# mKaloer/TFServingCache

Measured on AMD Instinct MI355X. Metric: predict req/sec (whole node), higher is better.
Workload: dtype bf16; 1 GPU; model=resnet50_v1.5, global_batch=8, seq_len=224, parallelism=ring-sharded serving x1, mode=headline (lru), full=False, batch_per_request=8, threads=10, n_models=1000, model_repo=hardlinked copies of one SavedModel per family (content-dedup applies), provider=disk, pool_size=10, n_cold_loads=872, transport=real gRPC (native nghttp2 front-end) over TCP loopback, client_channels=1, hipgraph=True

## Files before the change

### tfservingcache_amd/engine/csrc/executor.cpp

```cpp
#include <torch/extension.h>

#include <hip/hip_runtime.h>

#include <c10/hip/HIPStream.h>

#include <cstdint>
#include <stdexcept>
#include <vector>

#include "kernels.h"

namespace tfsc {

enum CallKind : int {
  K_ELT_UNARY = 0,
  K_ELT_BINARY,
  K_BN_ACT,
  K_SOFTMAX,
  K_LAYERNORM,
  K_MEAN_LAST,
  K_MEAN_MID,
  K_POOL,
  K_TRANSPOSE,
  K_GATHER,
  K_PAD_NHWC,
  K_GEMM,
  K_BGEMM,
  K_IM2COL,
  K_CONV,
  K_PAD_LAST,
  K_ATTENTION,
  K_DEPTHWISE,
  K_GEMM_FP8,
  K_QUANT_FP8,
  K_CAST,
  K_ARGMAX_LAST,
  K_SCATTER,
  K_RESIZE,
  K_ZERO_INSERT,
};
// ... 237 lines not shown
}

struct PtrDesc {
  uint8_t tag;
  int32_t reg = 0;
  int64_t off = 0;
};

class CallTemplate {
 public:
  std::vector<Call> calls;
  std::vector<std::vector<PtrDesc>> descs;

  ExecPlan* instantiate(uintptr_t ws,
                        const std::vector<uintptr_t>& bases) const {
    std::vector<Call> out = calls;
    for (size_t i = 0; i < out.size(); ++i) {
      auto& ds = descs[i];
      auto& ptrs = out[i].ptrs;
      ptrs.resize(ds.size());
      for (size_t j = 0; j < ds.size(); ++j) {
        const PtrDesc& d = ds[j];
        if (d.tag == 0)
          ptrs[j] = intptr_t(ws) + d.off;
        else if (d.tag == 1)
          ptrs[j] = intptr_t(bases.at(size_t(d.reg))) + d.off;
        else
          ptrs[j] = 0;
      }
    }
    return new ExecPlan(out);
  }
};

}

namespace py = pybind11;

void register_fastpath(py::module_& mod);
void register_frontend(py::module_& mod);
void register_rest_frontend(py::module_& mod);

PYBIND11_MODULE(TORCH_EXTENSION_NAME, mod) {
  using tfsc::Call;
  using tfsc::ExecPlan;

  py::class_<ExecPlan>(mod, "ExecPlan")
      .def(py::init([](py::list calls) {
        std::vector<Call> cs;
        cs.reserve(calls.size());
        for (auto item : calls) {
          py::tuple t = item.cast<py::tuple>();
          Call c;
          c.kind = t[0].cast<int>();
          c.ptrs = t[1].cast<std::vector<intptr_t>>();
          c.ints = t[2].cast<std::vector<int64_t>>();
          c.floats = t[3].cast<std::vector<float>>();
          cs.push_back(std::move(c));
        }
        return new ExecPlan(cs);
      }))
      .def("run", &ExecPlan::run, py::call_guard<py::gil_scoped_release>())
      .def("capture", &ExecPlan::capture,
           py::call_guard<py::gil_scoped_release>())
      .def("run_graph", &ExecPlan::run_graph,
           py::call_guard<py::gil_scoped_release>())
// ... 35 lines not shown
        t->calls.reserve(calls.size());
        t->descs.reserve(calls.size());
        for (auto item : calls) {
          py::tuple tu = item.cast<py::tuple>();
          Call c;
          c.kind = tu[0].cast<int>();
          std::vector<tfsc::PtrDesc> ds;
          for (auto dd : tu[1].cast<py::list>()) {
            py::tuple dt = dd.cast<py::tuple>();
            tfsc::PtrDesc d;
            d.tag = uint8_t(dt[0].cast<int>());
            if (d.tag == 0) {
              d.off = dt[1].cast<int64_t>();
            } else if (d.tag == 1) {
              d.reg = dt[1].cast<int32_t>();
              d.off = dt[2].cast<int64_t>();
            }
            ds.push_back(d);
          }
          c.ints = tu[2].cast<std::vector<int64_t>>();
          c.floats = tu[3].cast<std::vector<float>>();
          t->calls.push_back(std::move(c));
          t->descs.push_back(std::move(ds));
        }
        return t;
      }));

  mod.def("instantiate_plan",
          [](const tfsc::CallTemplate& t, uintptr_t ws,
             const std::vector<uintptr_t>& bases) {
            return std::unique_ptr<ExecPlan>(t.instantiate(ws, bases));
          });

  register_fastpath(mod);
  register_frontend(mod);
  register_rest_frontend(mod);

  mod.attr("ELT_ADD") = int(tfsc::ELT_ADD);
  mod.attr("ELT_SUB") = int(tfsc::ELT_SUB);
  mod.attr("ELT_MUL") = int(tfsc::ELT_MUL);
  mod.attr("ELT_DIV") = int(tfsc::ELT_DIV);
  mod.attr("ELT_MAX") = int(tfsc::ELT_MAX);
  mod.attr("ELT_MIN") = int(tfsc::ELT_MIN);
  mod.attr("ELT_SQDIFF") = int(tfsc::ELT_SQDIFF);
  mod.attr("ELT_RELU") = int(tfsc::ELT_RELU);
  mod.attr("ELT_TANH") = int(tfsc::ELT_TANH);
  mod.attr("ELT_SIGMOID") = int(tfsc::ELT_SIGMOID);
  mod.attr("ELT_ERF") = int(tfsc::ELT_ERF);
  mod.attr("ELT_SQRT") = int(tfsc::ELT_SQRT);
  mod.attr("ELT_RSQRT") = int(tfsc::ELT_RSQRT);
  mod.attr("ELT_EXP") = int(tfsc::ELT_EXP);
  mod.attr("ELT_NEG") = int(tfsc::ELT_NEG);
  mod.attr("ELT_SQUARE") = int(tfsc::ELT_SQUARE);
  mod.attr("ELT_GELU") = int(tfsc::ELT_GELU);
  mod.attr("ELT_RELU6") = int(tfsc::ELT_RELU6);

  mod.attr("ACT_NONE") = int(tfsc::ACT_NONE);
  mod.attr("ACT_RELU") = int(tfsc::ACT_RELU);
  mod.attr("ACT_TANH") = int(tfsc::ACT_TANH);
  mod.attr("ACT_SIGMOID") = int(tfsc::ACT_SIGMOID);
  mod.attr("ACT_GELU") = int(tfsc::ACT_GELU);
  mod.attr("ACT_RELU6") = int(tfsc::ACT_RELU6);
}
```

### tfservingcache_amd/engine/csrc/kernels.h

```cpp
#pragma once

#include <hip/hip_runtime.h>
#include <cstdint>

namespace tfsc {

enum EltFn : int {
  ELT_ADD = 0, ELT_SUB, ELT_MUL, ELT_DIV, ELT_MAX, ELT_MIN, ELT_SQDIFF,
  ELT_RELU, ELT_TANH, ELT_SIGMOID, ELT_ERF, ELT_SQRT, ELT_RSQRT, ELT_EXP,
  ELT_NEG, ELT_SQUARE, ELT_GELU, ELT_RELU6,
};

enum Act : int { ACT_NONE = 0, ACT_RELU, ACT_TANH, ACT_SIGMOID, ACT_GELU,
                 ACT_RELU6 };

constexpr int MAX_DIMS = 6;

struct BcastArgs {
  int ndim;
  int64_t dims[MAX_DIMS];
  int64_t sa[MAX_DIMS];
  int64_t sb[MAX_DIMS];
};

// ... 43 lines not shown
                 const ushort* bias, const ushort* residual, ushort* C,
                 int64_t M, int64_t N, int64_t K, int act, float alpha);

void launch_batched_gemm(hipStream_t s, const ushort* A, const ushort* B,
                         ushort* C, int64_t bat, int64_t M, int64_t N,
                         int64_t K, int64_t strideA, int64_t strideB,
                         int64_t strideC, bool trans_b, float alpha);

void launch_conv_igemm(hipStream_t s, const ushort* x, const ushort* w,
                       const ushort* bias, const ushort* residual,
                       const ushort* zeros, ushort* y,
                       int N, int H, int W, int C, int Kc, int R, int S,
                       int sh, int sw, int pt, int pl, int Ho, int Wo,
                       int k_pad, int act);

void launch_im2col(hipStream_t s, const ushort* x, ushort* y,
                   int N, int H, int W, int C, int R, int S,
                   int sh, int sw, int pt, int pl, int Ho, int Wo,
                   int k_pad);

void launch_depthwise_conv(hipStream_t s, const ushort* x, const ushort* w,
                           const ushort* bias, ushort* y,
                           int N, int H, int W, int C, int R, int S,
                           int sh, int sw, int pt, int pl, int Ho, int Wo,
                           int act);

void launch_resize_nhwc(hipStream_t s, const ushort* x, ushort* y, int N,
                        int H, int W, int C, int Ho, int Wo, int mode,
                        bool align_corners, bool half_pixel_centers);

void launch_zero_insert_nhwc(hipStream_t s, const ushort* x, ushort* y,
                             int N, int h, int w, int C, int sh, int sw);

void launch_gemm_fp8(hipStream_t s, const uint8_t* A, const float* sa,
                     const uint8_t* B, const float* sb,
                     const ushort* bias, const ushort* residual,
                     ushort* C, int64_t M, int64_t N, int64_t K,
                     int act);

void launch_quant_rowwise(hipStream_t s, const ushort* x, uint8_t* q,
                          float* scales, int64_t M, int64_t K,
                          int64_t Kp);

void launch_attention(hipStream_t s, const ushort* Q, const ushort* K,
                      const ushort* V, ushort* O, int B, int S, int H,
                      int D_, float scale, const ushort* bias = nullptr,
                      int64_t bias_sb = 0, int64_t bias_sh = 0,
                      int64_t bias_sq = 0);

}
```

### tfservingcache_amd/engine/csrc/ops/ops_memory.hip

```cpp
#include "../common.h"
#include "../kernels.h"

#include <stdexcept>
#include <string>

namespace tfsc {

constexpr int TPB = 256;
constexpr int MAX_BLOCKS = 2048;

static inline int grid_for(int64_t n, int per_thread = 1) {
  int64_t blocks = ceil_div(n, int64_t(TPB) * per_thread);
  return int(blocks < MAX_BLOCKS ? (blocks > 0 ? blocks : 1) : MAX_BLOCKS);
}

TFSC_DEV float apply_unary(float v, int fn) {
  switch (fn) {
    case ELT_RELU: return v > 0.f ? v : 0.f;
    case ELT_TANH: return tanhf(v);
    case ELT_SIGMOID: return 1.f / (1.f + __expf(-v));
    case ELT_ERF: return erff(v);
    case ELT_SQRT: return sqrtf(v);
    case ELT_RSQRT: return rsqrtf(v);
    case ELT_EXP: return __expf(v);
// ... 969 lines not shown
  int64_t stride = (int64_t)gridDim.x * TPB;
  for (int64_t i = i0; i < n_out; i += stride) {
    int c = int(i % C);
    int64_t t = i / C;
    int wo = int(t % Wo); t /= Wo;
    int ho = int(t % Ho); int n = int(t / Ho);
    ushort v = 0;
    if (ho % sh == 0 && wo % sw == 0)
      v = x[(((int64_t)n * h + ho / sh) * w + wo / sw) * C + c];
    y[i] = v;
  }
}

void launch_zero_insert_nhwc(hipStream_t s, const ushort* x, ushort* y,
                             int N, int h, int w, int C, int sh, int sw) {
  if (N <= 0 || h <= 0 || w <= 0 || C <= 0 || sh <= 0 || sw <= 0)
    throw std::runtime_error(
        "zero_insert: every dimension and stride must be positive");
  int64_t Ho64 = (int64_t)(h - 1) * sh + 1, Wo64 = (int64_t)(w - 1) * sw + 1;
  if (Ho64 > INT32_MAX || Wo64 > INT32_MAX)
    throw std::runtime_error("zero_insert: output image too large");
  int Ho = int(Ho64), Wo = int(Wo64);
  if (C % 8 == 0 && aligned16(x, y)) {
    int64_t n_grp = (int64_t)N * Ho * Wo * (C / 8);
    hipLaunchKernelGGL(k_zero_insert_v8, dim3(grid_for(n_grp)), dim3(TPB),
                       0, s, x, y, N, h, w, C, sh, sw, Ho, Wo);
    return;
  }
  int64_t n_out = (int64_t)N * Ho * Wo * C;
  hipLaunchKernelGGL(k_zero_insert, dim3(grid_for(n_out)), dim3(TPB), 0, s,
                     x, y, N, h, w, C, sh, sw, Ho, Wo);
}

}
```

### tfservingcache_amd/engine/emit.py

```python
from __future__ import annotations

from dataclasses import dataclass
from typing import Dict, List, Optional, Tuple

import numpy as np

from .planner import Plan, PlanOp

ALIGN = 256

WS = ("ws",)

KINDS = frozenset({
    "ELT_UNARY", "ELT_BINARY", "BN_ACT", "SOFTMAX", "LAYERNORM",
    "MEAN_LAST", "MEAN_MID", "POOL", "TRANSPOSE", "GATHER", "PAD_NHWC",
    "GEMM", "BGEMM", "CONV", "PAD_LAST", "ATTENTION", "DEPTHWISE",
    "GEMM_FP8", "QUANT_FP8", "CAST", "ARGMAX_LAST", "SCATTER", "RESIZE",
    "ZERO_INSERT",
})

_ROWWISE = {"softmax": "SOFTMAX", "reduce_mean_last": "MEAN_LAST",
            "argmax_last": "ARGMAX_LAST"}

_ACT_CODE = {"none": 0, "relu": 1, "tanh": 2, "sigmoid": 3, "gelu": 4,
             "relu6": 5}

_ELT_CODE = {
    "add": 0, "sub": 1, "mul": 2, "div": 3, "max": 4, "min": 5,
    "sqdiff": 6, "relu": 7, "tanh": 8, "sigmoid": 9, "erf": 10,
    "sqrt": 11, "rsqrt": 12, "exp": 13, "neg": 14, "square": 15,
    "gelu": 16, "relu6": 17,
}


# ... 53 lines not shown
def blob_layout(plan: Plan) -> BlobLayout:
    slots: Dict[int, Tuple[int, int]] = {}
    int_idx: List[int] = []
    total = 0
    for t in plan.tensors:
        if t.kind != "weight" or t.weight is None:
            continue
        if t.weight.dtype in _INT_DTYPES:
            int_idx.append(t.idx)
        else:
            n = int(t.weight.size)
            slots[t.idx] = (total, n)
            total += _pad128(n)
    return BlobLayout(slots, total, int_idx)


@dataclass
class Template:
    shapes: List[Tuple[int, ...]]
    root: List[int]
    bufs: Dict[int, _BufInfo]
    total_bytes: int
    scratch_off: Dict[int, int]
    region_keys: List[tuple]
    calls: List[tuple]


def build_template(plan: Plan, batch: int, dtype: str) -> Template:
    e = _Emitter(plan, batch, dtype)
    e.plan_buffers()
    e.emit_calls()
    return Template(e.shapes, e.root, e.bufs, e.total_bytes,
                    e.scratch_off, e.region_keys, e.calls)


class _Emitter:
    def __init__(self, plan: Plan, batch: int, dtype: str):
        self.plan = plan
        self.batch = batch
        self.dtype = dtype
        self.layout = blob_layout(plan)
        self.shapes: List[Tuple[int, ...]] = [
            plan.resolve_shape(t.shape, batch) for t in plan.tensors]
        self.root = [t.alias_of if t.alias_of is not None else t.idx
                     for t in plan.tensors]
        for i, r in enumerate(self.root):
            seen = 0
            while plan.tensors[r].alias_of is not None and seen < 16:
                r = plan.tensors[r].alias_of
                seen += 1
            self.root[i] = r
        self.region_keys: List[tuple] = []
        self._seen = set()
        self.calls: List[tuple] = []

    def _buf_bytes(self, idx: int) -> int:
        esize = 4 if self.plan.tensors[idx].dtype == "i32" else 2
        return max(_numel(self.shapes[idx]) * esize, esize)

    def plan_buffers(self) -> None:
        plan = self.plan
        root = self.root
        live_end: Dict[int, int] = {}
        scratch_sizes: Dict[int, int] = {}

        n_ops = len(plan.ops)
# ... 387 lines not shown
```

### tfservingcache_amd/engine/gpu.py

```python
from __future__ import annotations

import contextlib
import logging
import threading
from typing import Dict, List, Optional, Tuple

import warnings

import numpy as np

from .emit import (WS, _pad64, _pad128, _pad256b, blob_layout,
                   build_template)
from .planner import Plan, is_sym, resolve_dim

warnings.filterwarnings(
    "ignore", message="The given NumPy array is not writable")

log = logging.getLogger("tfsc.gpu")

_torch = None
_ext = None
_import_lock = threading.Lock()


class GpuUnavailable(RuntimeError):
    pass


class ModelReleasedError(RuntimeError):
    """Raised when a request races a pool eviction; callers re-fetch."""


def _load_backend():
    global _torch, _ext
    with _import_lock:
        if _ext is not None:
            return _torch, _ext
        import torch
        if not torch.cuda.is_available():
            raise GpuUnavailable("no ROCm GPU visible")
        try:
            from . import _tfsc_engine as ext
        except ImportError as e:
            raise GpuUnavailable(
                "GPU present but the tfsc HIP engine extension is not "
                "built — run `PYTORCH_ROCM_ARCH=gfx950 python setup.py "
                f"build_ext --inplace` ({e})") from e
        _torch, _ext = torch, ext
        return torch, ext


# ... 184 lines not shown
_arena_order: List[tuple] = []


def _get_ctx_template(plan, bucket: int, dtype: str):
    with _tmpl_lock:
        key = (id(plan), bucket, dtype)
        ent = _ctx_templates.get(key)
        if ent is None or ent[0] is not plan:
            return None
        _tmpl_order.remove(key)
        _tmpl_order.append(key)
        return ent[1]


def _put_ctx_template(plan, bucket: int, dtype: str, tmpl) -> None:
    with _tmpl_lock:
        key = (id(plan), bucket, dtype)
        if key not in _ctx_templates:
            _tmpl_order.append(key)
        _ctx_templates[key] = (plan, tmpl)
        while len(_tmpl_order) > _TMPL_CAP:
            old = _tmpl_order.pop(0)
            _ctx_templates.pop(old, None)


def _get_transform_arena(plan, dtype: str):
    with _tmpl_lock:
        key = (id(plan), dtype)
        ent = _transform_arenas.get(key)
        if ent is None or ent[0] is not plan:
            return None
        _arena_order.remove(key)
        _arena_order.append(key)
        return ent[1], ent[2]


def _put_transform_arena(plan, dtype: str, entries, pinned) -> None:
    with _tmpl_lock:
        key = (id(plan), dtype)
        if key in _transform_arenas:
            return
        _arena_order.append(key)
        _transform_arenas[key] = (plan, entries, pinned)
        while len(_arena_order) > _ARENA_CAP:
            old = _arena_order.pop(0)
            _transform_arenas.pop(old, None)


def _call_template(ext, tmpl):
    index = {k: i for i, k in enumerate(tmpl.region_keys)}
    return ext.CallTemplate([
        (getattr(ext, "K_" + kind),
         [(2,) if d is None else (0, d[1]) if d[0] == WS
          else (1, index[d[0]], d[1]) for d in descs],
         ints, floats)
        for kind, descs, ints, floats in tmpl.calls])


class ExecContext:

    def __init__(self, gm: "GpuModel", batch: int):
        self.gm = gm
        self.batch = batch
        torch, ext = _load_backend()
        plan = gm.plan
        dev = gm.device

        cached = _get_ctx_template(plan, batch, gm.dtype)
        if cached is None:
            tmpl = build_template(plan, batch, gm.dtype)
            ctmpl = _call_template(ext, tmpl)
        else:
            tmpl, ctmpl = cached
        self.shapes = tmpl.shapes
        self.root = tmpl.root
        self.bufs = tmpl.bufs
        self.total_bytes = tmpl.total_bytes
        self.scratch_off = tmpl.scratch_off
        self.workspace = torch.empty(self.total_bytes,
                                     dtype=torch.uint8, device=dev)
        n_before = gm.n_transforms()
        bases = gm.region_bases(tmpl.region_keys)
        self.exec_plan = ext.instantiate_plan(
            ctmpl, self.workspace.data_ptr(), bases)
        self._from_template = cached is not None and \
            gm.n_transforms() == n_before
        if cached is None:
            _put_ctx_template(plan, batch, gm.dtype, (tmpl, ctmpl))
            gm.publish_transform_arena()
        self.captured = False
        self._views: Dict[int, object] = {}
        self.lock = threading.Lock()
        self.fast_id: Optional[int] = None
        self.stream = torch.cuda.Stream(device=dev)
        self._pinned_in: Dict[int, object] = {}
        self._pinned_out: Dict[int, object] = {}
        self._pin_raws: List[object] = []

    def capture_only(self):
        torch, _ = _load_backend()
        with torch.cuda.device(self.gm.device), \
                torch.cuda.stream(self.stream):
            try:
                with capture_guard.capture():
                    self.exec_plan.capture()
            except Exception:
                log.exception("hipGraph capture failed; staying eager")
            self.captured = True

    def view(self, idx: int):
        torch, _ = _load_backend()
        r = self.root[idx]
        v = self._views.get(idx)
        if v is not None:
            return v
        info = self.bufs[r]
        t = self.gm.plan.tensors[r]
        base = self.workspace[info.offset:info.offset + info.nbytes]
        if t.dtype == "i32":
            v = base.view(torch.int32)[:int(np.prod(self.shapes[idx]))]
        else:
            v = base.view(torch.bfloat16)[:int(np.prod(self.shapes[idx]))]
        v = v.view(self.shapes[idx])
        self._views[idx] = v
        return v

    def run(self, feeds: Dict[int, np.ndarray],
            fetch: List[int]) -> Dict[int, np.ndarray]:
        if self.fast_id is not None and self.fast_id >= 0:
            self.gm._fast.lock_ctx(self.fast_id)
            try:
                return self._run_inner(feeds, fetch)
            finally:
                self.gm._fast.unlock_ctx(self.fast_id)
        return self._run_inner(feeds, fetch)

    def _run_inner(self, feeds: Dict[int, np.ndarray],
                   fetch: List[int]) -> Dict[int, np.ndarray]:
        torch, _ = _load_backend()
        with torch.cuda.device(self.gm.device), \
# ... 57 lines not shown

class GpuModel:

    BUCKETS = (1, 2, 4, 8, 16, 32, 64)

    def __init__(self, plan: Plan, device: str = "cuda:0",
                 max_batch: int = 64, use_graphs: bool = True,
                 n_streams: int = 6, model_name: str = "",
                 model_version: int = 0, dtype: str = "bf16"):
        torch, ext = _load_backend()
        if dtype not in ("bf16", "fp8"):
            raise ValueError(f"engine dtype {dtype!r} (bf16|fp8)")
        self.dtype = dtype
        self.plan = plan
        self.device = device
        self.model_name = model_name
        self.model_version = model_version
        self.n_streams = max(1, n_streams)
        self._fast = ext.FastModel(model_name or "model",
                                   int(model_version), self.n_streams)
        self.max_batch = max_batch
        self.use_graphs = use_graphs
        self._weights: Dict[int, object] = {}
        self._gemm_weights: Dict[Tuple[int, bool], object] = {}
        self._gemm_weights_fp8: Dict[Tuple[int, bool], tuple] = {}
        self._conv_weights: Dict[int, object] = {}
        self._contexts: Dict[int, List[ExecContext]] = {}
        self._lock = threading.Lock()
        self._released = False
        import os as _os
        import time as _time
        t0 = _time.monotonic()
        self._upload_pending = False
        with torch.cuda.device(device):
            self._upload_weights()
            restored = self.try_restore_transforms()
            if self._upload_pending or restored:
                with capture_guard.unsafe_host_op():
                    _get_upload_stream(torch, device).synchronize()
        if _os.environ.get("TFSC_LOAD_TIMING"):
            log.warning("upload_weights %.1fms (cached_blob=%s "
                        "arena=%s)", (_time.monotonic() - t0) * 1e3,
                        _blob_cache_get(plan) is not None, restored)

    def _upload_weights(self) -> None:
        torch, _ = _load_backend()
        layout = blob_layout(self.plan)
        tensors = self.plan.tensors
        self._int_idx = layout.int_idx
        for idx in layout.int_idx:
            self._weights[idx] = torch.from_numpy(np.ascontiguousarray(
                tensors[idx].weight.astype(np.int32))).to(self.device)
        float_ws = [(idx, tensors[idx].weight, off, n)
                    for idx, (off, n) in layout.slots.items()]
        total = layout.total
        if not float_ws:
            return
        import os as _os
        import time as _time
        timing = _os.environ.get("TFSC_LOAD_TIMING")
        ta = _time.monotonic()
        blob = torch.empty(total, dtype=torch.bfloat16, device=self.device)
        tb = _time.monotonic()
        cached = _blob_cache_get(self.plan)
        conv_held = False
        conv_lock = None
        if cached is None:
            conv_lock = _convert_lock(self.plan)
            conv_lock.acquire()
            conv_held = True
            cached = _blob_cache_get(self.plan)
            if cached is not None:
                conv_lock.release()
                conv_held = False
        try:
            self._upload_blob(torch, blob, cached, total, float_ws,
                              timing, ta, tb)
        finally:
            if conv_held:
                conv_lock.release()

    def _upload_blob(self, torch, blob, cached, total, float_ws,
                     timing, ta, tb):
        import time as _time
        if cached is not None and cached.numel() == total:
            up = _get_upload_stream(torch, self.device)
            tc = _time.monotonic()
            with capture_guard.unsafe_host_op():
                td = _time.monotonic()
                with torch.cuda.stream(up):
                    blob.copy_(cached, non_blocking=True)
                te = _time.monotonic()
                up.synchronize()
            if timing:
                tf_ = _time.monotonic()
                log.warning(
                    "upload phases: alloc=%.1f guard=%.1f copy=%.1f "
                    "sync=%.1f ms", (tb - ta) * 1e3, (td - tc) * 1e3,
                    (te - td) * 1e3, (tf_ - te) * 1e3)
        else:
            cpu_blob = None
            try:
                with capture_guard.unsafe_host_op():
                    cpu_blob = torch.empty(total, dtype=torch.bfloat16,
                                           pin_memory=True)
            except RuntimeError:
                log.warning("pinned weight-blob allocation failed; "
                            "skipping the converted-weight cache")
            with capture_guard.unsafe_host_op(), _staging_lock:
                stage = _get_staging(torch)
                cap = stage.numel()
                batch_items = []
                stage_off = 0

                def flush():
                    nonlocal stage_off
                    for s_off, b_off, n_ in batch_items:
                        blob[b_off:b_off + n_].copy_(
                            stage[s_off:s_off + n_], non_blocking=True)
                    torch.cuda.synchronize(self.device)
                    batch_items.clear()
                    stage_off = 0

                for _idx, w, off, n in float_ws:
                    src = torch.from_numpy(np.ascontiguousarray(
                        np.asarray(w, dtype=np.float32))).view(-1)
                    done = 0
                    while done < n:
                        if stage_off >= cap:
                            flush()
                        take = min(n - done, cap - stage_off)
                        stage[stage_off:stage_off + take].copy_(
                            src[done:done + take])
                        if cpu_blob is not None:
                            cpu_blob[off + done:off + done + take].copy_(
                                stage[stage_off:stage_off + take])
                        batch_items.append((stage_off, off + done, take))
                        stage_off += take
                        done += take
                flush()
            if cpu_blob is not None:
                _blob_cache_put(self.plan, cpu_blob)
        self._weight_blob = blob
        self._blob_slots = {idx: (off, n, tuple(w.shape))
                            for idx, w, off, n in float_ws}

    def master_weight(self, idx: int):
        t = self._weights.get(idx)
        if t is not None:
            return t
        slot = getattr(self, "_blob_slots", {}).get(idx)
        if slot is None:
            raise KeyError(f"no master weight for tensor {idx}")
        off, n, shape = slot
        t = self._weight_blob[off:off + n].view(shape)
        self._weights[idx] = t
        return t

    def has_master_weight(self, idx: int) -> bool:
        return idx in self._weights or \
            idx in getattr(self, "_blob_slots", {})

    def zeros_ptr(self) -> int:
        torch, _ = _load_backend()
        if getattr(self, "_zeros", None) is None:
            self._zeros = torch.zeros(64, dtype=torch.uint8,
                                      device=self.device)
        return self._zeros.data_ptr()

    def gemm_weight(self, idx: int, graph_trans_b: bool):
        torch, _ = _load_backend()
        key = (idx, graph_trans_b)
        wt = self._gemm_weights.get(key)
        if wt is not None:
            return wt
        av = self._arena_view(("gw",) + key)
        if av is not None:
            self._gemm_weights[key] = av
            return av
        if not self.has_master_weight(idx):
            raise RuntimeError(
                "GPU gemm requires a constant weight operand; "
                "activation x activation MatMul must be BatchMatMul")
        w = self.master_weight(idx).float()
        if not graph_trans_b:
            w = w.t().contiguous()
# ... 93 lines not shown
        return len(self._gemm_weights) + len(self._conv_weights) + \
            len(self._gemm_weights_fp8)

    def region_bases(self, keys) -> List[int]:
        arena = getattr(self, "_arena_dev", None)
        entries = self._arena_entries if arena is not None else {}
        arena_base = arena.data_ptr() if arena is not None else 0
        bases = []
        for key in keys:
            ent = entries.get(key)
            bases.append(arena_base + ent[1] if ent is not None
                         else self._region_ptr(key))
        return bases

    def _region_ptr(self, key: tuple) -> int:
        kind = key[0]
        if kind == "blob":
            return self._weight_blob.data_ptr()
        if kind == "zeros":
            return self.zeros_ptr()
        if kind == "int":
            return self._weights[key[1]].data_ptr()
        if kind == "gw":
            return self.gemm_weight(key[1], key[2]).data_ptr()
        if kind == "cw" and len(key) == 2:
            return self.conv_weight(key[1]).data_ptr()
        if kind == "cw" and key[2] == "cpad":
            return self.conv_weight_cpad(key[1], key[3]).data_ptr()
        if kind in ("f8q", "f8s"):
            q, scale = self.gemm_weight_fp8(key[1], key[2])
            return (q if kind == "f8q" else scale).data_ptr()
        raise KeyError(f"unknown weight region {key}")

    def publish_transform_arena(self) -> None:
        torch, _ = _load_backend()
        if _get_transform_arena(self.plan, self.dtype) is not None:
            return
        items = self._region_items()
        entries = []
        off = 0
        for key, t in items:
            nb = t.numel() * t.element_size()
            entries.append((key, off, nb, t.dtype, tuple(t.shape)))
            off = _pad256b(off + nb)
        if off == 0:
            return
        try:
            with capture_guard.unsafe_host_op():
                pinned = torch.empty(off, dtype=torch.uint8,
                                     pin_memory=True)
        except RuntimeError:
            log.warning("pinned transform-arena alloc failed; later "
                        "models will re-transform")
            return
        for (key, o, nb, dt, shape), (_k, t) in zip(entries, items):
            pinned[o:o + nb].view(dt)[:t.numel()].copy_(
                t.reshape(-1), non_blocking=False)
        _put_transform_arena(self.plan, self.dtype, entries, pinned)

    def try_restore_transforms(self) -> bool:
        torch, _ = _load_backend()
        got = _get_transform_arena(self.plan, self.dtype)
        if got is None:
            return False
        entries, pinned = got
        dev_arena = torch.empty(pinned.numel(), dtype=torch.uint8,
                                device=self.device)
        up = _get_upload_stream(torch, self.device)
        with capture_guard.unsafe_host_op():
            with torch.cuda.stream(up):
                dev_arena.copy_(pinned, non_blocking=True)
        self._arena_dev = dev_arena
        self._arena_entries = {tuple(e[0]): e for e in entries}
        for key, off, nb, dt, shape in entries:
            if key[0] == "int":
                self._weights[key[1]] = \
                    dev_arena[off:off + nb].view(dt).view(shape)
        return True

    def _arena_view(self, key: tuple):
        ent = getattr(self, "_arena_entries", {}).get(tuple(key))
        if ent is None or self._arena_dev is None:
            return None
        _key, off, nb, dt, shape = ent
        return self._arena_dev[off:off + nb].view(dt).view(shape)

    def weight_bytes(self) -> int:
        total = 0
        blob = getattr(self, "_weight_blob", None)
        if blob is not None:
            total += blob.numel() * blob.element_size()
        arena = getattr(self, "_arena_dev", None)
        if arena is not None:
            total += arena.numel() * arena.element_size()
        for d in (self._weights, self._gemm_weights, self._conv_weights):
            for wt in d.values():
                if wt is not None and getattr(wt, "untyped_storage",
                                              None) is not None:
                    total += wt.numel() * wt.element_size()
        return total

    def _bucket(self, batch: int) -> int:
        for b in self.BUCKETS:
            if b >= batch and b <= self.max_batch:
                return b
        return self.max_batch

    def streams_for(self, bucket: int) -> int:
        if bucket <= 4:
            return self.n_streams * 2
        return self.n_streams
# ... 82 lines not shown
            rows = v.shape[0] if v.ndim else 1
            row_elems = int(np.prod(v.shape[1:])) if v.ndim > 1 else 1
            raw = pinned_pool.alloc(torch, rows * row_elems * 4)
            ctx._pin_raws.append(raw)
            pin = _pin_view(torch, raw, (rows, row_elems), torch.float32)
            stage = torch.empty((rows, row_elems), dtype=torch.float32,
                                device=self.device)
            keep.extend([pin, stage])
            outs.append(ext.FastIO(alias, False, pin.data_ptr(),
                                   stage.data_ptr(), v.data_ptr(),
                                   row_elems, [int(d) for d in v.shape[1:]]))
        ctx._fast_keep = keep
        ctx.fast_id = self._fast.add_context(
            ctx.batch, self.streams_for(ctx.batch), ctx.exec_plan.ptr(),
            ctx.stream.cuda_stream, ins, outs)

    def prewarm(self, batch: int, limit: Optional[int] = None) -> None:
        plan = self.plan
        b = self._bucket(batch)
        want = self.streams_for(b) if limit is None \
            else min(limit, self.streams_for(b))
        feeds = {}
        for _alias, idx in plan.sig_inputs.items():
            shape = plan.resolve_shape(plan.tensors[idx].shape, b)
            dt = np.int32 if plan.tensors[idx].dtype == "i32" \
                else np.float32
            feeds[idx] = np.zeros(shape, dtype=dt)
        fetch = list(plan.sig_outputs.values())
        with self._lock:
            if self._released:
                raise ModelReleasedError(
                    "model was evicted from the GPU pool")
            ctxs = self._contexts.setdefault(b, [])
            while len(ctxs) < want:
                ctxs.append(ExecContext(self, b))
            todo = [c for c in ctxs if c.fast_id is None]
        for ctx in todo:
            with ctx.lock:
                if getattr(ctx, "_from_template", False) and \
                        self.use_graphs and not ctx.captured:
                    ctx.capture_only()
                else:
                    ctx.run(feeds, fetch)
                if ctx.fast_id is None and ctx.captured:
                    self._register_fast(ctx)

    def release(self) -> None:
        with self._lock:
            self._released = True
            ctx_lists = list(self._contexts.values())
            self._contexts.clear()
        try:
            self._fast.disable()
        except Exception:
            pass
        for ctxs in ctx_lists:
            for ctx in ctxs:
                ctx.lock.acquire()
                ctx.lock.release()
                ctx._pinned_in.clear()
                ctx._pinned_out.clear()
                ctx._fast_keep = None
                for raw in ctx._pin_raws:
                    pinned_pool.free(raw)
                ctx._pin_raws = []
        with self._lock:
            self._weights.clear()
            self._gemm_weights.clear()
            self._gemm_weights_fp8.clear()
            self._conv_weights.clear()
            self._arena_dev = None
            self._arena_entries = {}
            self._blob_slots = {}
            self._weight_blob = None
```

Baseline: 298.4 req/s.

## Restore cold-loaded models from a packed live-weight image with GPU scatter

On a cold model load, the code uploads one pinned image instead of the whole master weight blob. The image holds the transform arena plus only the weight slots the captured plan actually references, and a GPU kernel scatters those packed segments into their blob offsets. Large slots are copied directly. Any slot not in the live set is filled lazily by completing the blob upload on first access. The aim is to cut host-to-device bytes and per-load upload time on the many cold loads, at the cost of extra pinned host memory, more bookkeeping, and a possible stall when the lazy completion fires.

Measured after the change: 266.9 req/s. 0.894x the previous value.

```diff
diff --git a/tfservingcache_amd/engine/csrc/executor.cpp b/tfservingcache_amd/engine/csrc/executor.cpp
--- a/tfservingcache_amd/engine/csrc/executor.cpp
+++ b/tfservingcache_amd/engine/csrc/executor.cpp
@@ -6,6 +6,8 @@
 
 #include <cstdint>
 #include <stdexcept>
+#include <string>
+#include <utility>
 #include <vector>
 
 #include "kernels.h"
@@ -309,6 +311,92 @@
     return new ExecPlan(out);
   }
 };
+
+static void check_segments(const Segment* table, int64_t n_seg,
+                           int64_t src_limit, int64_t blob_nbytes) {
+  for (int64_t i = 0; i < n_seg; ++i) {
+    const Segment& g = table[i];
+    if (g.src < 0 || g.dst < 0 || g.nbytes <= 0 ||
+        ((g.src | g.dst | g.nbytes) & 15) ||
+        g.nbytes > src_limit || g.src > src_limit - g.nbytes ||
+        g.nbytes > blob_nbytes || g.dst > blob_nbytes - g.nbytes)
+      throw std::runtime_error("restore table: segment " +
+                               std::to_string(i) + " out of bounds");
+  }
+}
+
+static void hip_ok(hipError_t e, const char* what) {
+  if (e != hipSuccess)
+    throw std::runtime_error(std::string(what) + " failed: " +
+                             hipGetErrorString(e));
+}
+
+static void restore_image(uintptr_t image_host, uintptr_t image_dev,
+                          int64_t image_nbytes, int64_t table_off,
+                          int64_t n_seg, uintptr_t blob_host,
+                          uintptr_t blob_dev, int64_t blob_nbytes,
+                          const std::vector<std::pair<int64_t, int64_t>>&
+                              direct,
+                          uintptr_t stream) {
+  hipStream_t s = reinterpret_cast<hipStream_t>(stream);
+  if (!image_host || !image_dev || !blob_dev || image_nbytes <= 0 ||
+      blob_nbytes <= 0)
+    throw std::runtime_error("restore_image: null buffer");
+  if (n_seg < 0 || n_seg > INT32_MAX || table_off < 0 || (table_off & 15) ||
+      table_off > image_nbytes ||
+      n_seg * int64_t(sizeof(Segment)) > image_nbytes - table_off)
+    throw std::runtime_error("restore_image: table outside the image");
+  const Segment* table_host = reinterpret_cast<const Segment*>(
+      reinterpret_cast<const uint8_t*>(image_host) + table_off);
+  check_segments(table_host, n_seg, table_off, blob_nbytes);
+  for (const auto& d : direct) {
+    if (!blob_host || d.first < 0 || d.second <= 0 ||
+        d.second > blob_nbytes || d.first > blob_nbytes - d.second)
+      throw std::runtime_error("restore_image: direct copy out of bounds");
+  }
+  hip_ok(hipMemcpyAsync(reinterpret_cast<void*>(image_dev),
+                        reinterpret_cast<const void*>(image_host),
+                        size_t(image_nbytes), hipMemcpyHostToDevice, s),
+         "restore image upload");
+  for (const auto& d : direct)
+    hip_ok(hipMemcpyAsync(
+               reinterpret_cast<uint8_t*>(blob_dev) + d.first,
+               reinterpret_cast<const uint8_t*>(blob_host) + d.first,
+               size_t(d.second), hipMemcpyHostToDevice, s),
+           "direct slot upload");
+  if (n_seg > 0) {
+    launch_scatter_segments(
+        s, reinterpret_cast<const uint8_t*>(image_dev),
+        reinterpret_cast<uint8_t*>(blob_dev),
+        reinterpret_cast<const Segment*>(
+            reinterpret_cast<const uint8_t*>(image_dev) + table_off),
+        int(n_seg));
+    hip_ok(hipGetLastError(), "scatter_segments launch");
+  }
+  hip_ok(hipStreamSynchronize(s), "restore stream synchronize");
+}
+
+static void scatter_segments(uintptr_t image_dev, int64_t image_nbytes,
+                             uintptr_t blob_dev, int64_t blob_nbytes,
+                             uintptr_t table_dev, int64_t n_seg,
+                             uintptr_t stream) {
+  hipStream_t s = reinterpret_cast<hipStream_t>(stream);
+  if (!image_dev || !blob_dev || !table_dev || n_seg < 0 ||
+      n_seg > INT32_MAX)
+    throw std::runtime_error("scatter_segments: bad arguments");
+  std::vector<Segment> table(static_cast<size_t>(n_seg));
+  if (n_seg > 0)
+    hip_ok(hipMemcpy(table.data(), reinterpret_cast<const void*>(table_dev),
+                     table.size() * sizeof(Segment), hipMemcpyDeviceToHost),
+           "segment table read-back");
+  check_segments(table.data(), n_seg, image_nbytes, blob_nbytes);
+  launch_scatter_segments(s, reinterpret_cast<const uint8_t*>(image_dev),
+                          reinterpret_cast<uint8_t*>(blob_dev),
+                          reinterpret_cast<const Segment*>(table_dev),
+                          int(n_seg));
+  hip_ok(hipGetLastError(), "scatter_segments launch");
+  hip_ok(hipStreamSynchronize(s), "scatter stream synchronize");
+}
 
 }
 
@@ -410,6 +498,18 @@
             return std::unique_ptr<ExecPlan>(t.instantiate(ws, bases));
           });
 
+  mod.def("restore_image", &tfsc::restore_image,
+          py::arg("image_host"), py::arg("image_dev"),
+          py::arg("image_nbytes"), py::arg("table_off"), py::arg("n_seg"),
+          py::arg("blob_host"), py::arg("blob_dev"), py::arg("blob_nbytes"),
+          py::arg("direct"), py::arg("stream"),
+          py::call_guard<py::gil_scoped_release>());
+  mod.def("scatter_segments", &tfsc::scatter_segments,
+          py::arg("image_dev"), py::arg("image_nbytes"),
+          py::arg("blob_dev"), py::arg("blob_nbytes"),
+          py::arg("table_dev"), py::arg("n_seg"), py::arg("stream"),
+          py::call_guard<py::gil_scoped_release>());
+
   register_fastpath(mod);
   register_frontend(mod);
   register_rest_frontend(mod);
diff --git a/tfservingcache_amd/engine/csrc/kernels.h b/tfservingcache_amd/engine/csrc/kernels.h
--- a/tfservingcache_amd/engine/csrc/kernels.h
+++ b/tfservingcache_amd/engine/csrc/kernels.h
@@ -99,6 +99,15 @@
 void launch_zero_insert_nhwc(hipStream_t s, const ushort* x, ushort* y,
                              int N, int h, int w, int C, int sh, int sw);
 
+struct Segment {
+  int64_t src;
+  int64_t dst;
+  int64_t nbytes;
+};
+void launch_scatter_segments(hipStream_t s, const uint8_t* image_dev,
+                             uint8_t* blob_dev, const Segment* table_dev,
+                             int n_seg);
+
 void launch_gemm_fp8(hipStream_t s, const uint8_t* A, const float* sa,
                      const uint8_t* B, const float* sb,
                      const ushort* bias, const ushort* residual,
diff --git a/tfservingcache_amd/engine/csrc/ops/ops_memory.hip b/tfservingcache_amd/engine/csrc/ops/ops_memory.hip
--- a/tfservingcache_amd/engine/csrc/ops/ops_memory.hip
+++ b/tfservingcache_amd/engine/csrc/ops/ops_memory.hip
@@ -1025,4 +1025,35 @@
                      x, y, N, h, w, C, sh, sw, Ho, Wo);
 }
 
-}
+constexpr int SEG_BLOCKS_X = 32;
+
+__global__ void k_scatter_segments(const uint8_t* __restrict__ image,
+                                   uint8_t* __restrict__ blob,
+                                   const Segment* __restrict__ table) {
+  const Segment seg = table[blockIdx.y];
+  const uint4* src = reinterpret_cast<const uint4*>(image + seg.src);
+  uint4* dst = reinterpret_cast<uint4*>(blob + seg.dst);
+  int64_t n16 = seg.nbytes >> 4;
+  int64_t stride = (int64_t)gridDim.x * TPB;
+  for (int64_t i = (int64_t)blockIdx.x * TPB + threadIdx.x; i < n16;
+       i += stride)
+    dst[i] = src[i];
+}
+
+void launch_scatter_segments(hipStream_t s, const uint8_t* image_dev,
+                             uint8_t* blob_dev, const Segment* table_dev,
+                             int n_seg) {
+  if (n_seg < 0)
+    throw std::runtime_error("scatter_segments: negative segment count");
+  if ((reinterpret_cast<uintptr_t>(image_dev) |
+       reinterpret_cast<uintptr_t>(blob_dev)) & 15)
+    throw std::runtime_error("scatter_segments: bases must be 16-byte "
+                             "aligned");
+  for (int done = 0; done < n_seg; done += 65535) {
+    int n = n_seg - done < 65535 ? n_seg - done : 65535;
+    hipLaunchKernelGGL(k_scatter_segments, dim3(SEG_BLOCKS_X, n), dim3(TPB),
+                       0, s, image_dev, blob_dev, table_dev + done);
+  }
+}
+
+}
diff --git a/tfservingcache_amd/engine/emit.py b/tfservingcache_amd/engine/emit.py
--- a/tfservingcache_amd/engine/emit.py
+++ b/tfservingcache_amd/engine/emit.py
@@ -1,5 +1,6 @@
 from __future__ import annotations
 
+import bisect
 from dataclasses import dataclass
 from typing import Dict, List, Optional, Tuple
 
@@ -119,6 +120,47 @@
     e.emit_calls()
     return Template(e.shapes, e.root, e.bufs, e.total_bytes,
                     e.scratch_off, e.region_keys, e.calls)
+
+
+BLOB = ("blob",)
+
+
+def live_blob_slots(tmpl: Template, layout: BlobLayout) -> List[int]:
+    order = sorted((off * 2, (off + n) * 2, idx)
+                   for idx, (off, n) in layout.slots.items())
+    starts = [o[0] for o in order]
+    live = set()
+    for kind, descs, _ints, _floats in tmpl.calls:
+        for d in descs:
+            if d is None or d[0] != BLOB:
+                continue
+            i = bisect.bisect_right(starts, d[1]) - 1
+            if i < 0 or not order[i][0] <= d[1] < order[i][1]:
+                raise ValueError(
+                    f"{kind}: blob pointer at byte {d[1]} lies in no "
+                    "weight slot")
+            live.add(order[i][2])
+    return sorted(live)
+
+
+def pack_live_slots(layout: BlobLayout, live, base: int,
+                    direct_over: int):
+    if base % ALIGN:
+        raise ValueError("restore image base must be 256-byte aligned")
+    segments: List[Tuple[int, int, int]] = []
+    direct: List[Tuple[int, int]] = []
+    cursor = base
+    for idx in sorted(set(live), key=lambda i: layout.slots[i][0]):
+        off, n = layout.slots[idx]
+        dst, nbytes = off * 2, _pad128(n) * 2
+        if nbytes == 0:
+            continue
+        if nbytes > direct_over:
+            direct.append((dst, nbytes))
+        else:
+            segments.append((cursor, dst, nbytes))
+            cursor += nbytes
+    return segments, direct, cursor
 
 
 class _Emitter:
diff --git a/tfservingcache_amd/engine/gpu.py b/tfservingcache_amd/engine/gpu.py
--- a/tfservingcache_amd/engine/gpu.py
+++ b/tfservingcache_amd/engine/gpu.py
@@ -2,7 +2,9 @@
 
 import contextlib
 import logging
+import os
 import threading
+import time
 from typing import Dict, List, Optional, Tuple
 
 import warnings
@@ -10,13 +12,19 @@
 import numpy as np
 
 from .emit import (WS, _pad64, _pad128, _pad256b, blob_layout,
-                   build_template)
+                   build_template, live_blob_slots, pack_live_slots)
 from .planner import Plan, is_sym, resolve_dim
 
 warnings.filterwarnings(
     "ignore", message="The given NumPy array is not writable")
 
 log = logging.getLogger("tfsc.gpu")
+
+LIVE_RESTORE = os.environ.get(
+    "TFSC_LIVE_RESTORE", "on").lower() not in ("off", "0", "no")
+DIRECT_COPY_BYTES = 1 << 20
+POISON_FRESH_BLOB = False
+load_counts = {"first_or_full": 0, "image": 0, "completed_blob": 0}
 
 _torch = None
 _ext = None
@@ -267,19 +275,36 @@
             return None
         _arena_order.remove(key)
         _arena_order.append(key)
-        return ent[1], ent[2]
-
-
-def _put_transform_arena(plan, dtype: str, entries, pinned) -> None:
+        return ent[1], ent[2], ent[3]
+
+
+def _put_transform_arena(plan, dtype: str, entries, pinned, live=None,
+                         replace: bool = False) -> None:
     with _tmpl_lock:
         key = (id(plan), dtype)
         if key in _transform_arenas:
-            return
-        _arena_order.append(key)
-        _transform_arenas[key] = (plan, entries, pinned)
+            if not replace or _transform_arenas[key][0] is not plan:
+                return
+        else:
+            _arena_order.append(key)
+        _transform_arenas[key] = (plan, entries, pinned, live)
         while len(_arena_order) > _ARENA_CAP:
             old = _arena_order.pop(0)
             _transform_arenas.pop(old, None)
+
+
+class _LiveImage:
+    __slots__ = ("arena_bytes", "live", "n_seg", "table_off", "direct",
+                 "nbytes")
+
+    def __init__(self, arena_bytes, live, n_seg, table_off, direct,
+                 nbytes):
+        self.arena_bytes = arena_bytes
+        self.live = live
+        self.n_seg = n_seg
+        self.table_off = table_off
+        self.direct = direct
+        self.nbytes = nbytes
 
 
 def _call_template(ext, tmpl):
@@ -305,8 +330,10 @@
         if cached is None:
             tmpl = build_template(plan, batch, gm.dtype)
             ctmpl = _call_template(ext, tmpl)
+            live = frozenset(live_blob_slots(tmpl, gm.blob_layout()))
         else:
-            tmpl, ctmpl = cached
+            tmpl, ctmpl, live = cached
+        widened = gm.require_blob_slots(live)
         self.shapes = tmpl.shapes
         self.root = tmpl.root
         self.bufs = tmpl.bufs
@@ -321,8 +348,10 @@
         self._from_template = cached is not None and \
             gm.n_transforms() == n_before
         if cached is None:
-            _put_ctx_template(plan, batch, gm.dtype, (tmpl, ctmpl))
-            gm.publish_transform_arena()
+            _put_ctx_template(plan, batch, gm.dtype, (tmpl, ctmpl, live))
+            gm.publish_transform_arena(live)
+        elif widened:
+            gm.publish_transform_arena(live, extend_only=True)
         self.captured = False
         self._views: Dict[int, object] = {}
         self.lock = threading.Lock()
@@ -336,11 +365,16 @@
         torch, _ = _load_backend()
         with torch.cuda.device(self.gm.device), \
                 torch.cuda.stream(self.stream):
+            t0 = time.monotonic()
+            t1 = t0
             try:
                 with capture_guard.capture():
+                    t1 = time.monotonic()
                     self.exec_plan.capture()
             except Exception:
                 log.exception("hipGraph capture failed; staying eager")
+            self.gm._phase("cap_guard", (t1 - t0) * 1e3)
+            self.gm._phase("capture", (time.monotonic() - t1) * 1e3)
             self.captured = True
 
     def view(self, idx: int):
@@ -464,20 +498,130 @@
         import time as _time
         t0 = _time.monotonic()
         self._upload_pending = False
+        self._layout = None
+        self._blob_complete = True
+        self._blob_live: frozenset = frozenset()
+        self._blob_src = None
+        self._blob_lock = threading.Lock()
+        self.restored_from_image = False
+        self._timing = bool(_os.environ.get("TFSC_LOAD_TIMING"))
+        self._phases: Dict[str, float] = {}
         with torch.cuda.device(device):
-            self._upload_weights()
-            restored = self.try_restore_transforms()
-            if self._upload_pending or restored:
-                with capture_guard.unsafe_host_op():
-                    _get_upload_stream(torch, device).synchronize()
-        if _os.environ.get("TFSC_LOAD_TIMING"):
+            restored = self._restore_from_image()
+            if not restored:
+                self._upload_weights()
+                restored = self.try_restore_transforms()
+                if self._upload_pending or restored:
+                    ts0 = _time.monotonic()
+                    with capture_guard.unsafe_host_op():
+                        ts1 = _time.monotonic()
+                        _get_upload_stream(torch, device).synchronize()
+                    self._phase("guard", (ts1 - ts0) * 1e3)
+                    self._phase("sync", (_time.monotonic() - ts1) * 1e3)
+                load_counts["first_or_full"] += 1
+        self._phases["weights"] = (_time.monotonic() - t0) * 1e3
+        if self._timing:
             log.warning("upload_weights %.1fms (cached_blob=%s "
-                        "arena=%s)", (_time.monotonic() - t0) * 1e3,
-                        _blob_cache_get(plan) is not None, restored)
+                        "arena=%s image=%s)",
+                        (_time.monotonic() - t0) * 1e3,
+                        _blob_cache_get(plan) is not None, restored,
+                        self.restored_from_image)
+
+    def _phase(self, name: str, ms: float) -> None:
+        if self._timing:
+            self._phases[name] = self._phases.get(name, 0.0) + ms
+
+    def blob_layout(self):
+        if self._layout is None:
+            self._layout = blob_layout(self.plan)
+        return self._layout
+
+    def _restore_from_image(self) -> bool:
+        if not LIVE_RESTORE:
+            return False
+        torch, ext = _load_backend()
+        import time as _time
+        got = _get_transform_arena(self.plan, self.dtype)
+        if got is None or got[2] is None:
+            return False
+        entries, pinned, img = got
+        cached = _blob_cache_get(self.plan)
+        layout = self.blob_layout()
+        if cached is None or cached.numel() != layout.total or \
+                layout.total == 0:
+            return False
+        arena_keys = {tuple(e[0]) for e in entries}
+        if any(("int", idx) not in arena_keys for idx in layout.int_idx):
+            return False
+        ta = _time.monotonic()
+        blob = torch.empty(layout.total, dtype=torch.bfloat16,
+                           device=self.device)
+        dev_image = torch.empty(img.nbytes, dtype=torch.uint8,
+                                device=self.device)
+        up = _get_upload_stream(torch, self.device)
+        tb = _time.monotonic()
+        with capture_guard.unsafe_host_op():
+            tc = _time.monotonic()
+            if POISON_FRESH_BLOB:
+                blob.view(torch.int16).fill_(-1)
+                torch.cuda.current_stream(self.device).synchronize()
+            ext.restore_image(
+                pinned.data_ptr(), dev_image.data_ptr(), img.nbytes,
+                img.table_off, img.n_seg, cached.data_ptr(),
+                blob.data_ptr(), layout.total * 2, img.direct,
+                up.cuda_stream)
+        td = _time.monotonic()
+        self._weight_blob = blob
+        self._blob_slots = {
+            idx: (off, n, tuple(self.plan.tensors[idx].weight.shape))
+            for idx, (off, n) in layout.slots.items()}
+        self._int_idx = layout.int_idx
+        self._blob_complete = False
+        self._blob_live = img.live
+        self._blob_src = cached
+        self._adopt_arena(dev_image, entries)
+        self.restored_from_image = True
+        load_counts["image"] += 1
+        if self._timing:
+            self._phase("alloc", (tb - ta) * 1e3)
+            self._phase("guard", (tc - tb) * 1e3)
+            self._phase("copy_sync", (td - tc) * 1e3)
+            nbytes = img.nbytes + sum(n for _o, n in img.direct)
+            log.warning(
+                "restore image: bytes=%d segs=%d direct=%d alloc=%.1f "
+                "guard=%.1f copy+sync=%.1f ms", nbytes, img.n_seg,
+                len(img.direct), (tb - ta) * 1e3, (tc - tb) * 1e3,
+                (td - tc) * 1e3)
+        return True
+
+    def require_blob_slots(self, live) -> bool:
+        if self._blob_complete or live <= self._blob_live:
+            return False
+        self._complete_blob()
+        return True
+
+    def _complete_blob(self) -> None:
+        torch, _ = _load_backend()
+        with self._blob_lock:
+            if self._blob_complete:
+                return
+            blob, src = self._weight_blob, self._blob_src
+            if blob is None or src is None:
+                raise ModelReleasedError(
+                    "model was evicted from the GPU pool")
+            up = _get_upload_stream(torch, self.device)
+            with torch.cuda.device(self.device), \
+                    capture_guard.unsafe_host_op():
+                with torch.cuda.stream(up):
+                    blob.copy_(src, non_blocking=True)
+                up.synchronize()
+            self._blob_complete = True
+            self._blob_src = None
+            load_counts["completed_blob"] += 1
 
     def _upload_weights(self) -> None:
         torch, _ = _load_backend()
-        layout = blob_layout(self.plan)
+        layout = self.blob_layout()
         tensors = self.plan.tensors
         self._int_idx = layout.int_idx
         for idx in layout.int_idx:
@@ -526,6 +670,10 @@
                 up.synchronize()
             if timing:
                 tf_ = _time.monotonic()
+                self._phase("alloc", (tb - ta) * 1e3)
+                self._phase("guard", (td - tc) * 1e3)
+                self._phase("enqueue", (te - td) * 1e3)
+                self._phase("sync", (tf_ - te) * 1e3)
                 log.warning(
                     "upload phases: alloc=%.1f guard=%.1f copy=%.1f "
                     "sync=%.1f ms", (tb - ta) * 1e3, (td - tc) * 1e3,
@@ -584,6 +732,8 @@
         slot = getattr(self, "_blob_slots", {}).get(idx)
         if slot is None:
             raise KeyError(f"no master weight for tensor {idx}")
+        if not self._blob_complete and idx not in self._blob_live:
+            self._complete_blob()
         off, n, shape = slot
         t = self._weight_blob[off:off + n].view(shape)
         self._weights[idx] = t
@@ -743,9 +893,30 @@
             return (q if kind == "f8q" else scale).data_ptr()
         raise KeyError(f"unknown weight region {key}")
 
-    def publish_transform_arena(self) -> None:
+    def publish_transform_arena(self, live=frozenset(),
+                                extend_only: bool = False) -> None:
         torch, _ = _load_backend()
-        if _get_transform_arena(self.plan, self.dtype) is not None:
+        live = frozenset(live)
+        got = _get_transform_arena(self.plan, self.dtype)
+        src_blob = self._blob_src if self._blob_src is not None \
+            else _blob_cache_get(self.plan)
+        if src_blob is not None and \
+                src_blob.numel() != self.blob_layout().total:
+            src_blob = None
+        if got is not None:
+            entries, old, img = got
+            if img is None or live <= img.live or src_blob is None:
+                return
+            built = self._pack_image(img.arena_bytes, img.live | live,
+                                     src_blob)
+            if built is None:
+                return
+            pinned, new_img = built
+            pinned[:img.arena_bytes].copy_(old[:img.arena_bytes])
+            _put_transform_arena(self.plan, self.dtype, entries, pinned,
+                                 new_img, replace=True)
+            return
+        if extend_only:
             return
         items = self._region_items()
         entries = []
@@ -756,38 +927,79 @@
             off = _pad256b(off + nb)
         if off == 0:
             return
-        try:
-            with capture_guard.unsafe_host_op():
-                pinned = torch.empty(off, dtype=torch.uint8,
-                                     pin_memory=True)
-        except RuntimeError:
-            log.warning("pinned transform-arena alloc failed; later "
-                        "models will re-transform")
-            return
+        built = self._pack_image(off, live, src_blob) \
+            if src_blob is not None else None
+        if built is not None:
+            pinned, img = built
+        else:
+            img = None
+            try:
+                with capture_guard.unsafe_host_op():
+                    pinned = torch.empty(off, dtype=torch.uint8,
+                                         pin_memory=True)
+            except RuntimeError:
+                log.warning("pinned transform-arena alloc failed; later "
+                            "models will re-transform")
+                return
         for (key, o, nb, dt, shape), (_k, t) in zip(entries, items):
             pinned[o:o + nb].view(dt)[:t.numel()].copy_(
                 t.reshape(-1), non_blocking=False)
-        _put_transform_arena(self.plan, self.dtype, entries, pinned)
+        _put_transform_arena(self.plan, self.dtype, entries, pinned, img)
+
+    def _pack_image(self, arena_bytes: int, live, src_blob):
+        torch, _ = _load_backend()
+        segments, direct, end = pack_live_slots(
+            self.blob_layout(), live, arena_bytes, DIRECT_COPY_BYTES)
+        table_off = end
+        nbytes = _pad256b(table_off + 24 * len(segments))
+        try:
+            with capture_guard.unsafe_host_op():
+                pinned = torch.empty(max(nbytes, 256), dtype=torch.uint8,
+                                     pin_memory=True)
+        except RuntimeError:
+            log.warning("pinned restore-image alloc failed; later "
+                        "models upload the whole master blob")
+            return None
+        src_bytes = src_blob.view(torch.uint8)
+        for src, dst, nb in segments:
+            pinned[src:src + nb].copy_(src_bytes[dst:dst + nb])
+        if segments:
+            table = torch.tensor(segments, dtype=torch.int64).reshape(-1)
+            pinned[table_off:table_off + 24 * len(segments)].view(
+                torch.int64).copy_(table)
+        return pinned, _LiveImage(arena_bytes, frozenset(live),
+                                  len(segments), table_off, direct,
+                                  pinned.numel())
 
     def try_restore_transforms(self) -> bool:
         torch, _ = _load_backend()
+        import time as _time
         got = _get_transform_arena(self.plan, self.dtype)
         if got is None:
             return False
-        entries, pinned = got
-        dev_arena = torch.empty(pinned.numel(), dtype=torch.uint8,
+        entries, pinned, img = got
+        arena_bytes = img.arena_bytes if img is not None \
+            else pinned.numel()
+        dev_arena = torch.empty(arena_bytes, dtype=torch.uint8,
                                 device=self.device)
         up = _get_upload_stream(torch, self.device)
+        t0 = _time.monotonic()
         with capture_guard.unsafe_host_op():
+            t1 = _time.monotonic()
             with torch.cuda.stream(up):
-                dev_arena.copy_(pinned, non_blocking=True)
+                dev_arena.copy_(pinned[:arena_bytes], non_blocking=True)
+        self._phase("guard", (t1 - t0) * 1e3)
+        self._phase("enqueue", (_time.monotonic() - t1) * 1e3)
+        self._adopt_arena(dev_arena, entries)
+        return True
+
+    def _adopt_arena(self, dev_arena, entries) -> None:
         self._arena_dev = dev_arena
         self._arena_entries = {tuple(e[0]): e for e in entries}
         for key, off, nb, dt, shape in entries:
             if key[0] == "int":
                 self._weights[key[1]] = \
                     dev_arena[off:off + nb].view(dt).view(shape)
-        return True
 
     def _arena_view(self, key: tuple):
         ent = getattr(self, "_arena_entries", {}).get(tuple(key))
@@ -936,8 +1148,10 @@
                 raise ModelReleasedError(
                     "model was evicted from the GPU pool")
             ctxs = self._contexts.setdefault(b, [])
+            t0 = time.monotonic()
             while len(ctxs) < want:
                 ctxs.append(ExecContext(self, b))
+            self._phase("context", (time.monotonic() - t0) * 1e3)
             todo = [c for c in ctxs if c.fast_id is None]
         for ctx in todo:
             with ctx.lock:
@@ -945,9 +1159,18 @@
                         self.use_graphs and not ctx.captured:
                     ctx.capture_only()
                 else:
+                    t0 = time.monotonic()
                     ctx.run(feeds, fetch)
+                    self._phase("warm_run", (time.monotonic() - t0) * 1e3)
                 if ctx.fast_id is None and ctx.captured:
+                    t0 = time.monotonic()
                     self._register_fast(ctx)
+                    self._phase("fast_reg", (time.monotonic() - t0) * 1e3)
+        if self._timing and self._phases:
+            log.warning("load phases: image=%s %s", self.restored_from_image,
+                        " ".join(f"{k}={v:.2f}" for k, v in
+                                 sorted(self._phases.items())))
+            self._phases = {}
 
     def release(self) -> None:
         with self._lock:
@@ -977,3 +1200,4 @@
             self._arena_entries = {}
             self._blob_slots = {}
             self._weight_blob = None
+            self._blob_src = None
```
